# NicolaDM/MAPLE

Measured on AMD Instinct MI355X. Metric: candidate SPR placements/sec, higher is better.
Workload: dtype f64

## Files before the change

### include/maple_hip.h

```cpp
#ifndef MAPLE_HIP_H
#define MAPLE_HIP_H
#include <stdint.h>

#ifdef __cplusplus
extern "C" {
#endif

#define MAPLE_ABI_VERSION 4

enum {
    MAPLE_OK = 0,
    MAPLE_ERR_ARG = -1,
    MAPLE_ERR_HIP = -2,
    MAPLE_ERR_NOMEM = -3,
    MAPLE_ERR_STATE = -4,
    MAPLE_ERR_FATAL = -5
};

#define MAPLE_META_TYPE(m)   ((m) & 7u)
#define MAPLE_META_REF(m)    (((m) >> 3) & 3u)
#define MAPLE_META_HASD0     (1u << 5)
#define MAPLE_META_HASD1     (1u << 6)
#define MAPLE_META_FLAG      (1u << 7)
#define MAPLE_META_AUXOFF(m) ((m) >> 8)
// ... 4 lines not shown
    double thresholdProb;
    double minBLenSensitivity;
    double thresholdDiffForUpdate;
    double thresholdFoldChangeUpdate;
    double defaultBLen;
} maple_params;

int maple_abi_version(void);
int maple_create(maple_ctx **out, int device, int32_t lRef, const uint8_t *refIdx,
                 const double *rootFreqs4, const maple_params *params, uint64_t arena_bytes);
int maple_destroy(maple_ctx *ctx);
typedef struct {
    uint32_t structSize;
    int32_t wavePerItemMax;
    int32_t placementChunkMax;
    int32_t noCladeScan;
    int32_t verbose;
    int32_t wideOutsideFrontier;
    int32_t denseWideScoring;
    int32_t waveAllBelow;
    int32_t noOverHint;
    int32_t noAheadExpansion;
    int32_t noAheadSpeculation;
} maple_tuning;
int maple_set_tuning(maple_ctx *ctx, const maple_tuning *t);
const char *maple_last_error(maple_ctx *ctx);

int maple_set_model(maple_ctx *ctx, const double *Q16, const double *siteRates, int usingErrorRate,
                    double errorRateGlobal, const double *errorRates);
int maple_get_model(maple_ctx *ctx, double *cumulativeRate , double *cumulativeErrorRate ,
                    double *totError);

int maple_lists_update(maple_ctx *ctx, int32_t n, const int32_t *ids, const int64_t *ent_off, const int32_t *pos,
                       const uint32_t *meta, const int64_t *aux_off, const double *aux);
int maple_lists_upload(maple_ctx *ctx, int32_t n_lists, const int64_t *ent_off, const int32_t *pos,
                       const uint32_t *meta, const int64_t *aux_off, const double *aux, int32_t *first_id);
int maple_lists_sizes(maple_ctx *ctx, int32_t n, const int32_t *ids, int32_t *n_ent, int32_t *n_aux);
int maple_lists_download(maple_ctx *ctx, int32_t n, const int32_t *ids, const int64_t *ent_off, int32_t *pos,
                         uint32_t *meta, const int64_t *aux_off, double *aux);
int maple_arena_mark(maple_ctx *ctx, int64_t *mark);
int maple_arena_release(maple_ctx *ctx, int64_t mark);
int maple_arena_stats(maple_ctx *ctx, int64_t *n_lists, int64_t *n_entries, int64_t *n_aux, int64_t *cap_entries);
int maple_arena_compact(maple_ctx *ctx, int64_t nLive, const int32_t *live, int32_t *newIds);

int maple_mutations_upload(maple_ctx *ctx, int32_t n_lists, const int64_t *off, const int32_t *mut3,
                           int32_t *first_id);
// ... 110 lines not shown
```

### include/maple_hip_debug.h

```cpp
#ifndef MAPLE_HIP_DEBUG_H
#define MAPLE_HIP_DEBUG_H
#include "maple_hip.h"

#ifdef __cplusplus
extern "C" {
#endif

int maple_debug_frontier_levels(maple_ctx *ctx, int32_t cap, int64_t *itemsUpdating, int64_t *itemsCached, float *msUpdating,
                                float *msCached, int32_t *n, int64_t *waveItemsSmall , int64_t *waveItemsBig );

int maple_debug_wave_append_batch(maple_ctx *ctx, int32_t n, const int32_t *parentList, const int32_t *childList,
                                  const uint8_t *isTipC, const double *bLen, double *outLK, float *ms);
int maple_debug_trace_query(maple_ctx *ctx, int32_t query);
int maple_debug_calib_walk(maple_ctx *ctx, uint64_t bytes, int32_t repeats, float *ms);
int maple_debug_calib_write(maple_ctx *ctx, uint64_t bytes, int32_t mode, int32_t repeats, float *ms);
int maple_debug_trace_read(maple_ctx *ctx, int32_t *n, int32_t *items4 , double *vals2 );
int maple_debug_gpv_batch(maple_ctx *ctx, int32_t n, const int32_t *i12, const double *totLen, const double *M16,
                          const double *errorRate, const double *vect4, const uint8_t *upNode, const uint8_t *flag,
                          double *out4);
int maple_debug_simplify_batch(maple_ctx *ctx, int32_t n, const double *vec4, const int32_t *refA, int32_t *out);
int maple_debug_frontier_pass_batch(maple_ctx *ctx, int32_t n, const int32_t *list, const int32_t *mutList, const uint8_t *dirIsUp,
                                    int32_t waveForm, int32_t *outList, uint8_t *grade, uint8_t *sameHandle);

#ifdef __cplusplus
}
#endif
#endif
```

### maple_amd/csrc/debug_abi.hip

```cpp
#include "../../include/maple_hip_debug.h"
#include "genome_dev.h"
#include "ctx_host.h"
#include "batch_host.h"
#include "frontier.h"
#include "frontier_dev.h"

#include <algorithm>

using namespace frt;

__global__ __launch_bounds__(MAPLE_BLOCK) void k_calib_walk(const unsigned long long *buf, long long nLists, unsigned long long *sink)
{
    unsigned long long acc = 0;
    for (long long l = (long long)blockIdx.x * blockDim.x + threadIdx.x; l < nLists; l += (long long)gridDim.x * blockDim.x) {
        const unsigned long long *p = buf + l * 64;
        unsigned idx = 0;
        for (int k = 0; k < 64; k++) {
            unsigned long long w = p[idx];
            acc += w;
            idx = (idx + 1 + (unsigned)(w & 0)) & 63;
        }
    }
    if (acc == 0x123456789abcdefull) *sink = acc;
}
// ... 146 lines not shown

extern "C" int maple_debug_trace_query(maple_ctx *c, int32_t query)
{
    if (!c) return MAPLE_ERR_ARG;
    c->trace_query = query;
    if (query >= 0) {
        HIPCK(c, c->s_trace_i.reserve(4 * 4096 + 4));
        HIPCK(c, c->s_trace_d.reserve(2 * 4096));
        HIPCK(c, hipMemset(c->s_trace_i.p, 0, (4 * 4096 + 4) * sizeof(int32_t)));
    }
    return MAPLE_OK;
}

extern "C" int maple_debug_trace_read(maple_ctx *c, int32_t *n, int32_t *items4, double *vals2)
{
    if (!c || !n || !items4 || !vals2 || !c->s_trace_i.p) return MAPLE_ERR_ARG;
    HIPCK(c, hipMemcpy(n, c->s_trace_i.p + 4 * 4096, sizeof(int32_t), hipMemcpyDeviceToHost));
    HIPCK(c, hipMemcpy(items4, c->s_trace_i.p, 4 * 4096 * sizeof(int32_t), hipMemcpyDeviceToHost));
    HIPCK(c, hipMemcpy(vals2, c->s_trace_d.p, 2 * 4096 * sizeof(double), hipMemcpyDeviceToHost));
    return MAPLE_OK;
}

extern "C" int maple_debug_frontier_levels(maple_ctx *c, int32_t cap, int64_t *itemsUpdating, int64_t *itemsCached, float *msUpdating,
                                           float *msCached, int32_t *n, int64_t *waveItemsSmall, int64_t *waveItemsBig)
{
    if (!c || cap < 0 || !itemsUpdating || !itemsCached || !msUpdating || !msCached || !n) return MAPLE_ERR_ARG;
    HIPCK(c, hipSetDevice(c->device));
    int nn = 0;
    const int rc = frontier_level_profile(c, cap, (long long *)itemsUpdating, (long long *)itemsCached, msUpdating, msCached, &nn,
                                          (long long *)waveItemsSmall, (long long *)waveItemsBig);
    *n = nn;
    return rc;
}

template <bool RV, bool U, bool SS>
__global__ __launch_bounds__(FR_BLOCK) void k_debug_fpass_lane(const DevModel *__restrict__ mp, ArenaViewS av, FPools fp, int n, const int32_t *l,
                                                               const int32_t *ml, const uint8_t *up, int32_t *handle)
{
    __shared__ Lds lds;
    const DevModel &m = *mp;
    stage_model(m, lds);
    Ctx<RV, U, SS> c(m, lds);
    const long long laneId = (long long)blockIdx.x * blockDim.x + threadIdx.x;
    for (long long i = laneId; i < n; i += (long long)gridDim.x * blockDim.x)
        handle[i] = fpass_removed(c, fp, av, laneId, ftree(l[i]), ml[i], up[i] != 0);
}

template <bool RV, bool U, bool SS>
__global__ __launch_bounds__(FR_BLOCK) void k_debug_fpass_wave(const DevModel *__restrict__ mp, ArenaViewS av, FPools fp, int n, const int32_t *l,
                                                               const int32_t *ml, const uint8_t *up, int32_t *handle)
{
    __shared__ Lds lds;
    const DevModel &m = *mp;
// ... 95 lines not shown
```

### maple_amd/csrc/frontier.h

```cpp
#pragma once
#include "ctx_host.h"

#define FR_STATUS_FALLBACK (-8)

struct FrontierStats {
    int levels = 0, overflow = 0;
    long long itemsUpdating = 0, itemsCached = 0, tempLists = 0, tempWords = 0, tempAux = 0, records = 0;
};

struct FrontierWide {
    const int32_t *rowOf;
    const double *cacheS;
    FiniteRows fin;
    hipEvent_t rowsReady;
    int forceWide;
    const int32_t *frameParent = nullptr, *frameNode = nullptr;
    int nFrames = 0;
};

__attribute__((visibility("hidden")))
int frontier_search(maple_ctx *c, const SearchParams &P, int m, const int32_t *nodes, int budget, int zeroBudget, SearchOut *hostOut,
                    uint2 *poolW, double *poolA, unsigned long long *poolUsed, long long poolCapW, long long poolCapA,
                    FrontierStats *stats, long long itemsHint, const FrontierWide *wide = nullptr,
                    const uint8_t *overHint = nullptr);
__attribute__((visibility("hidden"))) void frontier_scratch_free(maple_ctx *c);
__attribute__((visibility("hidden"))) int frontier_export(maple_ctx *c, long long cap, int32_t *q, int32_t *node, long long *n);
__attribute__((visibility("hidden")))
int frontier_level_profile(maple_ctx *c, int cap, long long *itemsU, long long *itemsC, float *msU, float *msC, int *n,
                           long long *waveSmall = nullptr, long long *waveBig = nullptr);
```

### maple_amd/csrc/frontier.hip

```cpp
#include "ctx_host.h"
#include "frontier_dev.h"

#include <chrono>

using namespace frt;

namespace {

__global__ __launch_bounds__(FR_BLOCK) void k_fr_arena_recs(ArenaViewS av, int n, LRec *out)
{
    for (int i = blockIdx.x * blockDim.x + threadIdx.x; i < n; i += gridDim.x * blockDim.x)
        out[i] = lrec_make(av.ent_off[i], av.n_ent[i], av.aux_off[i], av.n_aux[i]);
}

template <bool RV, bool U, bool SS>
__global__ __launch_bounds__(FR_BLOCK) void k_fr_begin(const DevModel *__restrict__ mp, ArenaViewS av, DevTree T, SearchParams P, int n,
                                                       const int32_t *nodes, FPools fp, SearchOut *out, int budget, int zeroBudget,
                                                       const int32_t *rowOf, int forceWide, const uint8_t *overHint)
{
    __shared__ Lds lds;
    const DevModel &m = *mp;
    stage_model(m, lds);
    Ctx<RV, U, SS> c(m, lds);
    for (int q = blockIdx.x * blockDim.x + threadIdx.x; q < n; q += gridDim.x * blockDim.x) {
// ... 63 lines not shown
        const int pp = rp.up;
        const NodeRec rpp = T.nd[pp];
        const bool first = rpp.c0 == parent;
        const double d = rs.dist + rp.dist;
        int pv1 = ftree(rs.lower), rprUp = rpr, vUpUp = ftree(first ? rpp.upRight : rpp.upLeft), rprDown = rpr;
        if (fp.mat) {
            pv1 = fpass_store(fp, av, c.m.lRef, laneId, pv1, rs.mutId, true);
            if (rp.mutId >= 0) {
                pv1 = fvalid(pv1) ? fpass_store(fp, av, c.m.lRef, laneId, pv1, rp.mutId, true) : pv1;
                rprUp = fpass_removed(c, fp, av, laneId, rpr, rp.mutId, true);
            }
            vUpUp = fpass_store(fp, av, c.m.lRef, laneId, vUpUp, rp.mutId, false);
            if (rs.mutId >= 0) {
                vUpUp = fvalid(vUpUp) ? fpass_store(fp, av, c.m.lRef, laneId, vUpUp, rs.mutId, false) : vUpUp;
                rprDown = hBest;
            }
            if (pv1 == -2 || vUpUp == -2 || !fvalid(rprUp) || !fvalid(rprDown)) { S.state = FS_FALLBACK; continue; }
        }
        S.seed0 = fpush(fp, budget, q, true, pp, first ? 1 : 2, pv1, d, curLK, 0, rprUp, curLK);
        S.seed1 = fpush(fp, budget, q, true, S.sibling, 0, vUpUp, d, curLK, 0, rprDown, curLK);
    }
}

#define FR_LVL 8
__global__ void k_fr_snap_u(FCtr *ctr, long long capU, long long capR, long long capPassR, unsigned long long *lvl, int maxLevels)
{
    if (threadIdx.x == 0 && blockIdx.x == 0) {
        ctr->loU = ctr->hiU; ctr->hiU = min(ctr->usedU, (unsigned long long)capU);
        atomicExch(&ctr->safePassR, min(ctr->nPassR, (unsigned long long)capPassR));
        __threadfence();
        atomicExch(&ctr->safeR, min(ctr->usedR, (unsigned long long)capR));
        ctr->bigUsed = 0;
        const unsigned long long heavySmall = ctr->permHeavy, heavyBig = ctr->permHeavy2;
        ctr->permDown = ctr->permUp = ctr->permDownB = ctr->permUpB = ctr->permHeavy = ctr->permHeavy2 = 0;
        if (lvl) {
            const int l = ctr->nLevels++;
            if (l < maxLevels) { lvl[FR_LVL * l] = ctr->loU; lvl[FR_LVL * l + 1] = ctr->hiU; lvl[FR_LVL * l + 6] = lvl[FR_LVL * l + 7] = 0; }
            if (l > 0 && l - 1 < maxLevels) { lvl[FR_LVL * (l - 1) + 6] = heavySmall; lvl[FR_LVL * (l - 1) + 7] = heavyBig; }
        }
    }
}
__global__ void k_fr_snap_c(FCtr *ctr, long long capCC, long long capPass, long long capDeferred, unsigned long long *lvl, int maxLevels)
{
    if (threadIdx.x == 0 && blockIdx.x == 0) {
        ctr->loC = ctr->hiC; ctr->hiC = min(ctr->usedC, (unsigned long long)capCC);
        ctr->loR = ctr->hiR; ctr->hiR = atomicAdd(&ctr->safeR, 0ull);
// ... 248 lines not shown
                atomicAdd(&fp.ctr->dbgC[2], (unsigned long long)(tp2 - tp1)); atomicAdd(&fp.ctr->dbgC[3], (unsigned long long)(tp3 - tp2));
                atomicAdd(&fp.ctr->dbgC[4], (unsigned long long)len); atomicAdd(&fp.ctr->dbgC[5], (unsigned long long)nS);
                atomicAdd(&fp.ctr->dbgC[6], (unsigned long long)tot);
            }
        }
#endif
    }
    for (int off = 32; off > 0; off >>= 1) {
        nSc += ((unsigned long long)(uint32_t)__shfl_down((int)(nSc >> 32), off, 64) << 32) | (uint32_t)__shfl_down((int)nSc, off, 64);
        bSc += ((unsigned long long)(uint32_t)__shfl_down((int)(bSc >> 32), off, 64) << 32) | (uint32_t)__shfl_down((int)bSc, off, 64);
    }
    if ((threadIdx.x & 63) == 0 && nSc) { atomicAdd(&fp.ctr->scoredC, nSc); atomicAdd(&fp.ctr->bytesC, bSc); }
}

__device__ __forceinline__ long long fidx(const FPools &fp, int ref) { return ref >= 0 ? fp.capU + ref : -(long long)(ref + 2); }
__device__ __forceinline__ int fsize(const FPools &fp, int ref) { return ref == FR_NONE ? 0 : fp.lsize[fidx(fp, ref)]; }

__device__ __forceinline__ void fr_layer(const FPools &fp, int level, int which, long long &lo1, long long &n1, long long &lo2, long long &n2)
{
    const unsigned long long *L = fp.lvl + (size_t)FR_LVL * level;
    if (which == 0) { lo1 = (long long)L[0]; n1 = (long long)L[1] - lo1; lo2 = 0; n2 = 0; }
    else { lo1 = (long long)L[2]; n1 = (long long)L[3] - lo1; lo2 = (long long)L[4]; n2 = (long long)L[5] - lo2; }
}
__global__ __launch_bounds__(FR_BLOCK) void k_fr_layout_sizes(FPools fp, int level, int which)
{
    long long lo1, n1, lo2, n2;
    fr_layer(fp, level, which, lo1, n1, lo2, n2);
    const long long n = n1 + n2;
    const bool isU = which == 0;
    for (long long i = (long long)blockIdx.x * blockDim.x + threadIdx.x; i < n; i += (long long)gridDim.x * blockDim.x) {
        const long long at = i < n1 ? lo1 + i : lo2 + (i - n1);
        const FItem &it = isU ? fp.U[at] : fp.C[at];
        fp.lsize[isU ? at : fp.capU + at] = 1 + fsize(fp, it.child0) + fsize(fp, it.child1);
    }
}
__global__ __launch_bounds__(FR_BLOCK) void k_fr_layout_totals(int n, FPools fp)
{
    for (int q = blockIdx.x * blockDim.x + threadIdx.x; q < n; q += gridDim.x * blockDim.x) {
        const FSearch &S = fp.S[q];
        fp.tot[q] = S.state == FS_ACTIVE ? fsize(fp, S.seed0) + fsize(fp, S.seed1) : 0;
    }
}
__global__ __launch_bounds__(1024) void k_fr_layout_scan(int n, const int32_t *in, long long *out)
{
    __shared__ long long part[1024];
    const int t = threadIdx.x, per = (n + 1023) / 1024;
    const int lo = min(n, t * per), hi = min(n, lo + per);
    long long s = 0;
    for (int i = lo; i < hi; i++) s += in[i];
    part[t] = s;
    __syncthreads();
    if (t == 0) {
        long long run = 0;
        for (int i = 0; i < 1024; i++) { const long long v = part[i]; part[i] = run; run += v; }
        out[n] = run;
    }
    __syncthreads();
    long long run = part[t];
    for (int i = lo; i < hi; i++) { out[i] = run; run += in[i]; }
}
__global__ __launch_bounds__(FR_BLOCK) void k_fr_layout_seeds(int n, FPools fp)
{
    for (int q = blockIdx.x * blockDim.x + threadIdx.x; q < n; q += gridDim.x * blockDim.x) {
        const FSearch &S = fp.S[q];
        if (S.state != FS_ACTIVE || fp.vbase[q + 1] > fp.capVisit) continue;
        long long p = fp.vbase[q];
        if (S.seed1 != FR_NONE) { const long long x = fidx(fp, S.seed1); fp.lpos[x] = (int32_t)p; fp.lpar[x] = -1; p += fp.lsize[x]; }
        if (S.seed0 != FR_NONE) { const long long x = fidx(fp, S.seed0); fp.lpos[x] = (int32_t)p; fp.lpar[x] = -1; }
    }
}
__global__ __launch_bounds__(FR_BLOCK) void k_fr_layout_place(FPools fp, int level, int which)
{
    long long lo1, n1, lo2, n2;
    fr_layer(fp, level, which, lo1, n1, lo2, n2);
    const long long n = n1 + n2;
    const bool isU = which == 0;
    for (long long i = (long long)blockIdx.x * blockDim.x + threadIdx.x; i < n; i += (long long)gridDim.x * blockDim.x) {
        const long long at = i < n1 ? lo1 + i : lo2 + (i - n1);
        const long long own = isU ? at : fp.capU + at;
        const int p = fp.lpos[own];
        if (p < 0) continue;
        const FItem &it = isU ? fp.U[at] : fp.C[at];
        FVisit v;
        v.midProb = it.midProb; v.lastLK = it.lastLK; v.ref = isU ? -((int)at + 2) : (int)at; v.size = fp.lsize[own];
        v.parent = fp.lpar[own]; v.flags = it.flags; v.dir = it.dir; v.failsOut = 0;
        fp.visit[p] = v;
        int q = p + 1;
        if (it.child1 != FR_NONE) { const long long x = fidx(fp, it.child1); fp.lpos[x] = q; fp.lpar[x] = p; q += fp.lsize[x]; }
        if (it.child0 != FR_NONE) { const long long x = fidx(fp, it.child0); fp.lpos[x] = q; fp.lpar[x] = p; }
    }
}

__device__ inline void fr_replay_done(const SearchParams &P, const FPools &fp, SearchOut *out, int q, FSearch &S, int slHead, int nApp, bool handBack,
                                      const int *hShort = nullptr, int nShort = 0, int reason = 0)
{
    for (int k = 0; k < nShort; k++) if (hShort[k] == S.hRpr0 && !handBack) { handBack = true; reason = 4; }
    if (handBack) { S.state = FS_FALLBACK; out[q].status = FR_STATUS_FALLBACK; atomicAdd(&fp.ctr->fbReason[reason & 7], 1); return; }
    S.slHead = slHead; S.nApp = nApp;
    int cnt = 0;
    for (int r = slHead; r != FR_NONE; r = item_of(fp, r).next)
        if (item_of(fp, r).midProb >= S.curLK - P.thrOptTopo) cnt++;
    const unsigned long long base = atomicAdd(&fp.ctr->nRecs, (unsigned long long)cnt);
    if ((long long)(base + cnt) > fp.capRecs) {
        S.state = FS_FALLBACK; out[q].status = FR_STATUS_FALLBACK; fp.ctr->overflow = 1;
        for (long long k2 = (long long)base; k2 < fp.capRecs; k2++) { fp.recs[k2].q = q; fp.recs[k2].ref = FR_NONE; }
        return;
    }
    S.recBase = (int32_t)base; S.recCount = cnt;
    int k = 0;
    for (int r = slHead; r != FR_NONE; r = item_of(fp, r).next)
        if (item_of(fp, r).midProb >= S.curLK - P.thrOptTopo) {
            FRec &x = fp.recs[base + k++];
// ... 449 lines not shown
__global__ __launch_bounds__(FR_BLOCK) void k_fr_export(FPools fp, long long nU, long long nC, long long nR, int32_t *outQ, int32_t *outNode)
{
    const long long n = nU + nC + nR;
    for (long long i = (long long)blockIdx.x * blockDim.x + threadIdx.x; i < n; i += (long long)gridDim.x * blockDim.x) {
        const FItem &it = i < nU ? fp.U[i] : (i < nU + nC ? fp.C[i - nU] : fp.C[fp.capCC + (i - nU - nC)]);
        outQ[i] = it.q; outNode[i] = it.t1;
    }
}

struct FrontierScratch {
    DevBuf<uint8_t> itemsU, itemsC, srch, recs, ctr;
    DevBuf<uint2> tw, sw, bw;
    DevBuf<double> ta, sa, sais, ba;
    DevBuf<LRec> trec, arec;
    DevBuf<int32_t> nodes, expQ, expNode;
    DevBuf<uint8_t> out, wideBr, tflag, overHint;
    DevBuf<int32_t> wideRow, wideQ, wideCtr, perm, perm2, perm3, perm4, tot, lsize, lpos, lpar, passList, passListR, deferred;
    DevBuf<uint2> bw2; DevBuf<double> ba2;
    DevBuf<uint8_t> visit;
    DevBuf<unsigned long long> lvl;
    DevBuf<long long> vbase;
    std::vector<unsigned long long> lastLvl;
    std::vector<size_t> lastSlotsU, lastSlotsC;
    long long lastU = -1, lastC = -1, lastR = 0;
    long long needR = 0;
    long long needU = 0, needC = 0, needL = 0, needW = 0, needA = 0, needM = 0;
    bool lastOverflow = false;
    FPools lastPools{};
    int capE = 0;
    hipStream_t side = nullptr, side2 = nullptr;
    hipEvent_t evFork = nullptr, evJoin = nullptr, evFork2 = nullptr, evJoin2 = nullptr;
};

}

void frontier_scratch_free(maple_ctx *c)
{
    FrontierScratch *F = (FrontierScratch *)c->frontier;
    if (!F) return;
    F->itemsU.release(); F->itemsC.release(); F->srch.release(); F->recs.release(); F->ctr.release();
    F->tw.release(); F->sw.release(); F->ta.release(); F->sa.release(); F->sais.release(); F->bw.release(); F->ba.release();
    F->trec.release(); F->arec.release(); F->nodes.release(); F->out.release();
    F->expQ.release(); F->expNode.release();
    F->perm.release(); F->perm2.release(); F->perm3.release(); F->perm4.release(); F->tot.release(); F->lsize.release(); F->lpos.release(); F->lpar.release(); F->visit.release(); F->lvl.release(); F->vbase.release(); F->wideBr.release(); F->wideRow.release(); F->wideQ.release(); F->wideCtr.release(); F->passList.release(); F->passListR.release(); F->deferred.release(); F->overHint.release(); F->bw2.release(); F->ba2.release(); F->tflag.release();
    if (F->evFork) (void)hipEventDestroy(F->evFork);
    if (F->evJoin) (void)hipEventDestroy(F->evJoin);
// ... 261 lines not shown
        launchesC++;
        return MAPLE_OK;
    };
    auto bail = [&](int rc) { (void)hipStreamSynchronize(s); (void)hipStreamSynchronize(s2); (void)hipStreamSynchronize(s3); return rc; };
    k_fr_snap_u<<<1, 64, 0, s>>>(fp.ctr, fp.capU, fp.capC - fp.capCC, fp.capPassR, fp.lvl, fp.maxLevels);
    if (hipGetLastError() != hipSuccess || hipEventRecord(F.evFork, s) != hipSuccess || hipStreamWaitEvent(s2, F.evFork, 0) != hipSuccess
        || (anyWide && wide->rowsReady && hipStreamWaitEvent(s2, wide->rowsReady, 0) != hipSuccess))
        return bail(fail(c, MAPLE_ERR_HIP, "frontier level loop: HIP error"));
    const int groupLevels = m <= 64 ? 2 : 8;
    for (;;) {
        for (int g = 0; g < groupLevels; g++) {
            { const int rc_ = u_level(); if (rc_) return bail(rc_); }
            for (int k2 = 0; k2 < 2; k2++) { const int rc_ = c_launch(); if (rc_) return bail(rc_); }
        }
        if (hipGetLastError() != hipSuccess || hipMemcpyAsync(&hc, fp.ctr, sizeof(FCtr), hipMemcpyDeviceToHost, s) != hipSuccess
            || hipStreamSynchronize(s) != hipSuccess)
            return bail(fail(c, MAPLE_ERR_HIP, "frontier level loop: HIP error"));
        if (hc.hiU == hc.loU) break;
        if (levels > 100000) return bail(fail(c, MAPLE_ERR_FATAL, "frontier search did not terminate"));
    }
    for (;;) {
        for (int g = 0; g < groupLevels; g++) { const int rc_ = c_launch(); if (rc_) return bail(rc_); }
        if (passQueued && hipStreamWaitEvent(s2, F.evJoin2, 0) != hipSuccess) return bail(fail(c, MAPLE_ERR_HIP, "frontier level loop: HIP error"));
        if (hipGetLastError() != hipSuccess || hipMemcpyAsync(&hc, fp.ctr, sizeof(FCtr), hipMemcpyDeviceToHost, s2) != hipSuccess
            || hipStreamSynchronize(s2) != hipSuccess)
            return bail(fail(c, MAPLE_ERR_HIP, "frontier level loop: HIP error"));
        const unsigned long long haveC = std::min<unsigned long long>(hc.usedC, (unsigned long long)fp.capCC),
                                 haveR = std::min<unsigned long long>(hc.usedR, (unsigned long long)(fp.capC - fp.capCC));
        if (hc.hiC == haveC && hc.hiR == haveR && hc.hiD == std::min<unsigned long long>(hc.nDeferred, (unsigned long long)fp.capDeferred)) break;
        if (launchesC > 200000) return bail(fail(c, MAPLE_ERR_FATAL, "frontier search did not terminate"));
    }
    if (hipEventRecord(F.evJoin, s2) != hipSuccess || hipStreamWaitEvent(s, F.evJoin, 0) != hipSuccess)
        return bail(fail(c, MAPLE_ERR_HIP, "frontier level loop: HIP error"));
    if (dbgTime) fprintf(stderr, "[maple]   frontier +%.1f ms: expansion done (%d updating levels, %d cached launches)\n", sinceEnter(), levels, launchesC);
    size_t slotWide = (size_t)-1;
    auto finishStage = [&]() -> int {
    if (anyWide) {
        hipEvent_t w0, w1;
        TRY(maple_internal_ev_pair(c, &w0, &w1, MAPLE_K_FR_WIDE, 0.0, 0.0));
        slotWide = c->ev_used / 2 - 1;
        const int capB = 512, gridW = (int)std::min<size_t>(8192, wideIdx.size());
        HIPCK(c, F.wideBr.reserve_exact(std::max(F.wideBr.cap, (size_t)gridW * capB * sizeof(BestRec))));
        HIPCK(c, hipEventRecord(F.evFork, s));
        HIPCK(c, hipStreamWaitEvent(s2, F.evFork, 0));
        HIPCK(c, hipEventRecord(w0, s2));
        const size_t dyn = (size_t)Tw.scanDepthCap * (sizeof(double) + sizeof(int) + sizeof(unsigned));
        k_fr_replay_wide<<<gridW, 64, dyn, s2>>>(Tw, P, (int)wideIdx.size(), F.wideQ.p, F.wideRow.p, wide->cacheS, wide->fin, fp, dout,
                                                  (BestRec *)F.wideBr.p, capB, F.wideCtr.p);
        HIPCK(c, hipGetLastError());
        HIPCK(c, hipEventRecord(w1, s2));
        HIPCK(c, hipEventRecord(F.evJoin, s2));
    }
    TRY(maple_internal_ev_pair(c, &er0, &er1, MAPLE_K_FR_REPLAY, (double)m, 0.0));
    HIPCK(c, hipEventRecord(er0, s));
    const int gridLayout = (int)std::min<long long>(1024, std::max<long long>(64, (long long)m / 64));
    if (levels <= fp.maxLevels && launchesC <= fp.maxLevels && fp.visit) {
        HIPCK(c, hipMemsetAsync(fp.lpos, 0xFF, (size_t)fp.capVisit * sizeof(int32_t), s));
        for (int l = launchesC - 1; l >= 0; l--) k_fr_layout_sizes<<<gridLayout, FR_BLOCK, 0, s>>>(fp, l, 1);
        for (int l = levels - 1; l >= 0; l--) k_fr_layout_sizes<<<gridLayout, FR_BLOCK, 0, s>>>(fp, l, 0);
        k_fr_layout_totals<<<gridN, FR_BLOCK, 0, s>>>(m, fp);
        k_fr_layout_scan<<<1, 1024, 0, s>>>(m, fp.tot, fp.vbase);
        k_fr_layout_seeds<<<gridN, FR_BLOCK, 0, s>>>(m, fp);
        for (int l = 0; l < levels; l++) k_fr_layout_place<<<gridLayout, FR_BLOCK, 0, s>>>(fp, l, 0);
        for (int l = 0; l < launchesC; l++) k_fr_layout_place<<<gridLayout, FR_BLOCK, 0, s>>>(fp, l, 1);
        HIPCK(c, hipGetLastError());
        TRY(stage("k_fr_layout"));
    } else fp.visit = nullptr;
    k_fr_replay<<<gridN, FR_BLOCK, 0, s>>>(P, m, fp, dout);
    TRY(stage("k_fr_replay"));
    if (anyWide) HIPCK(c, hipStreamWaitEvent(s, F.evJoin, 0));
    if (anyWide && fp.mat && wide->nFrames > 0) {
        DISPATCH3(c, k_fr_wide_frames, <<<std::min(gridUpd, 512), FR_BLOCK, 0, s>>>(c->d_model, av, T, fp, wide->frameParent, wide->frameNode));
        TRY(stage("k_fr_wide_frames"));
    }
    DISPATCH3(c, k_fr_refine, <<<gridUpd, FR_BLOCK, 0, s>>>(c->d_model, av, T, fp));
    TRY(stage("k_fr_refine"));
    k_fr_finish<<<gridN, FR_BLOCK, 0, s>>>(av, T, P, m, fp, dout, poolW, poolA, poolUsed, poolCapW, poolCapA);
    HIPCK(c, hipGetLastError());
    HIPCK(c, hipEventRecord(er1, s));
    HIPCK(c, hipEventRecord(e1, s));
    HIPCK(c, hipMemcpyAsync(hostOut, dout, (size_t)m * sizeof(SearchOut), hipMemcpyDeviceToHost, s));
    HIPCK(c, hipMemcpyAsync(&hc, fp.ctr, sizeof(FCtr), hipMemcpyDeviceToHost, s));
    HIPCK(c, hipStreamSynchronize(s));
    return MAPLE_OK;
    };
    { const int rc_ = finishStage(); if (rc_) return bail(rc_); }
    if (dbgTime) fprintf(stderr, "[maple]   frontier +%.1f ms: replay, refinement, final selection done; results on the host\n", sinceEnter());
    if (dbgTime && (hc.fbReason[0] | hc.fbReason[1] | hc.fbReason[2] | hc.fbReason[3] | hc.fbReason[4] | hc.fbReason[5] | hc.fbReason[6] | hc.fbReason[7]))
        fprintf(stderr, "[maple]   exact walk handed searches to the one-lane kernel: %d a merge within tolerance, %d a list re-expressed from a shortened one, "
                        "%d a fifth shortened list, %d the search's own first list shortened, %d marked list without a layout, %d other; whole-tree searches: "
                        "%d short list / scan slots / marked item list, %d a scanned branch whose list shorten() would change\n",
                hc.fbReason[1], hc.fbReason[2], hc.fbReason[3], hc.fbReason[4], hc.fbReason[5], hc.fbReason[0], hc.fbReason[6], hc.fbReason[7]);
    if (dbgTime && hc.overflow)
        fprintf(stderr, "[maple]   frontier pools, asked / capacity: updating items %llu / %lld, cached items %llu / %lld, roots %llu / %lld, temporary lists %llu / %lld "
                        "(words %llu / %lld, aux %llu / %lld), pass entries %llu / %lld, of roots %llu / %lld, records %llu / %lld\n",
                hc.usedU, fp.capU, hc.usedC, fp.capCC, hc.usedR, fp.capC - fp.capCC, hc.nLists, fp.capL, hc.usedW, fp.capW, hc.usedA, fp.capA,
                hc.nPass, fp.capPass, hc.nPassR, fp.capPassR, hc.nRecs, fp.capRecs);
    {
        const double meanCand = c->n_scored ? c->scored_bytes_total / c->n_scored : 0.0;
        double units = 0.0, bytes = 0.0;
        double unitsW = 0.0, bytesW = 0.0;
        for (int k = 0; k < m; k++) {
            if (hostOut[k].status != 0 && hostOut[k].status != -1) continue;
            if (anyWide && wide->rowOf[k] >= 0) {
                const int32_t l = c->h_tree_lower[nodes[k]];
                unitsW += hostOut[k].nAppend;
                bytesW += 8.0 * hostOut[k].nAppend + (l >= 0 ? 8.0 * c->h_n_ent[l] + 8.0 * c->h_n_aux[l] : 0.0);
                continue;
            }
            units += hostOut[k].nAppend;
// ... 21 lines not shown
    {
        const char *nm[4] = {"small class", "512 class", "small class, one lane (a list does not fit)", "512 class, one lane (a list does not fit)"};
        for (int b = 0; b < 4; b++)
            if (hc.dbgWCnt[b]) fprintf(stderr, "[maple] wavefront-wide updating items, %s: %llu items, mean %.3f ms, slowest %.3f ms\n", nm[b],
                                       hc.dbgWCnt[b], hc.dbgWT[b] * 1e-5 / hc.dbgWCnt[b], hc.dbgWMax[b] * 1e-5);
    }
    if (anyWide) {
        double tw = 0, ts = 0, mw = 0, ms = 0; long long ns = 0, mxn = 0;
        for (int k : wideIdx) {
            tw += hostOut[k].tStep * 1e-5; ts += hostOut[k].tReplay * 1e-5; ns += hostOut[k].nSteps;
            mw = std::max(mw, hostOut[k].tStep * 1e-5); ms = std::max(ms, hostOut[k].tReplay * 1e-5); mxn = std::max<long long>(mxn, hostOut[k].nSteps);
        }
        fprintf(stderr, "[maple] wide replay profile over %zu searches: item walk %.1f ms total (max %.2f), scans %.1f ms total (max %.2f), %lld scans (max %lld)\n",
                wideIdx.size(), tw, mw, ts, ms, ns, mxn);
    }
#endif
    if (!(anyWide && wide->forceWide) && (m >= 1024 || m >= F.needM)) {
        F.needU = (long long)hc.usedU; F.needC = (long long)hc.usedC; F.needR = (long long)hc.usedR; F.needL = (long long)hc.nLists; F.needW = (long long)hc.usedW;
        F.needA = (long long)hc.usedA; F.needM = m; F.lastOverflow = hc.overflow != 0;
    }
    F.lastU = std::min((long long)hc.usedU, fp.capU); F.lastC = std::min((long long)hc.usedC, fp.capCC);
    F.lastR = std::min((long long)hc.usedR, fp.capC - fp.capCC); F.lastPools = fp;
    {
        const int nl = std::min(std::max(levels, launchesC), fp.maxLevels);
        F.lastLvl.assign((size_t)nl * FR_LVL, 0ull);
        if (nl) HIPCK(c, hipMemcpy(F.lastLvl.data(), fp.lvl, (size_t)nl * FR_LVL * sizeof(unsigned long long), hipMemcpyDeviceToHost));
        for (int l = 0; l < nl; l++) {
            unsigned long long *L = F.lastLvl.data() + (size_t)FR_LVL * l;
            if (l >= levels) L[0] = L[1] = L[6] = L[7] = 0;
            if (l >= launchesC) L[2] = L[3] = L[4] = L[5] = 0;
        }
        F.lastSlotsU = slotsU; F.lastSlotsC = slotsC;
    }
    if (hc.overflow) F.lastU = F.lastC = -1;
    if (stats) {
        stats->levels = levels; stats->itemsUpdating = (long long)hc.usedU; stats->itemsCached = (long long)(hc.usedC + hc.usedR);
        stats->tempLists = (long long)hc.nLists; stats->tempWords = (long long)hc.usedW; stats->tempAux = (long long)hc.usedA;
        stats->records = (long long)hc.nRecs; stats->overflow = hc.overflow;
    }
    return MAPLE_OK;
}

int frontier_export(maple_ctx *c, long long cap, int32_t *q, int32_t *node, long long *n)
{
    FrontierScratch *F = (FrontierScratch *)c->frontier;
    if (!F || F->lastU < 0) return fail(c, MAPLE_ERR_STATE, "no complete frontier search to export");
    const long long tot = F->lastU + F->lastC + F->lastR;
    *n = tot;
    if (tot > cap) return fail(c, MAPLE_ERR_ARG, "%lld expanded items do not fit in %lld", tot, cap);
    if (tot == 0) return MAPLE_OK;
    HIPCK(c, F->expQ.reserve((size_t)tot));
    HIPCK(c, F->expNode.reserve((size_t)tot));
    k_fr_export<<<(int)std::min<long long>(1024, (tot + FR_BLOCK - 1) / FR_BLOCK), FR_BLOCK, 0, c->stream>>>(F->lastPools, F->lastU, F->lastC, F->lastR,
                                                                                                          F->expQ.p, F->expNode.p);
    HIPCK(c, hipGetLastError());
    HIPCK(c, hipMemcpyAsync(q, F->expQ.p, (size_t)tot * sizeof(int32_t), hipMemcpyDeviceToHost, c->stream));
    HIPCK(c, hipMemcpyAsync(node, F->expNode.p, (size_t)tot * sizeof(int32_t), hipMemcpyDeviceToHost, c->stream));
    HIPCK(c, hipStreamSynchronize(c->stream));
    return MAPLE_OK;
}

int frontier_level_profile(maple_ctx *c, int cap, long long *itemsU, long long *itemsC, float *msU, float *msC, int *n, long long *waveSmall,
                           long long *waveBig)
{
    FrontierScratch *F = (FrontierScratch *)c->frontier;
    if (!F) return fail(c, MAPLE_ERR_STATE, "no frontier search to report on");
    const int nl = (int)(F->lastLvl.size() / FR_LVL);
    *n = nl;
    for (int l = 0; l < nl && l < cap; l++) {
        const unsigned long long *L = F->lastLvl.data() + (size_t)FR_LVL * l;
        itemsU[l] = (long long)(L[1] - L[0]);
        itemsC[l] = (long long)(L[3] - L[2]) + (long long)(L[5] - L[4]);
        if (waveSmall) waveSmall[l] = (long long)L[6];
        if (waveBig) waveBig[l] = (long long)L[7];
        msU[l] = msC[l] = 0.f;
        const size_t su = l < (int)F->lastSlotsU.size() ? F->lastSlotsU[l] : (size_t)-1 / 4, sc = l < (int)F->lastSlotsC.size() ? F->lastSlotsC[l] : (size_t)-1 / 4;
        if (2 * su + 1 < c->ev_used) { HIPCK(c, hipEventSynchronize(c->evs[2 * su + 1])); HIPCK(c, hipEventElapsedTime(&msU[l], c->evs[2 * su], c->evs[2 * su + 1])); }
        if (2 * sc + 1 < c->ev_used) { HIPCK(c, hipEventSynchronize(c->evs[2 * sc + 1])); HIPCK(c, hipEventElapsedTime(&msC[l], c->evs[2 * sc], c->evs[2 * sc + 1])); }
    }
    return MAPLE_OK;
}
```

### maple_amd/runtime.py

```python
from __future__ import annotations

import ctypes as C
import os

import numpy as np

from .genome_list import PackedLists, pack_lists, pack_mutations, unpack_list

HERE = os.path.dirname(os.path.abspath(__file__))
LIB_PATH = os.path.join(HERE, "libmaple_hip.so")

EXPORTS = [
    "maple_abi_version", "maple_create", "maple_destroy", "maple_set_tuning", "maple_last_error", "maple_set_model", "maple_get_model",
    "maple_lists_upload", "maple_lists_update", "maple_lists_sizes", "maple_lists_download", "maple_arena_mark", "maple_arena_release",
    "maple_arena_stats", "maple_mutations_upload", "maple_append_batch", "maple_merge_batch", "maple_blen_batch",
    "maple_differ_batch", "maple_pass_branch_batch", "maple_shorten_batch", "maple_root_vector_batch",
    "maple_evaluate_placement_batch", "maple_update_partials", "maple_update_partials_touched", "maple_tree_patch", "maple_append_batch_dev", "maple_append_queries_dev", "maple_timing_reset", "maple_timing_read", "maple_timing_read_each",
    "maple_append_algorithmic_bytes", "maple_tree_upload", "maple_spr_search_batch", "maple_minor_batch", "maple_root_prob_batch", "maple_candset_create", "maple_append_candset",
    "maple_minor_candset", "maple_placement_search_batch", "maple_placement_prepare", "maple_placement_ahead", "maple_placement_ahead_stats", "maple_set_fatal_policy",
    "maple_timing_read_kind", "maple_placement_supports_batch",
    "maple_candset_destroy", "maple_spr_search_visited", "maple_arena_compact", "maple_append_queries_argmax_dev", "maple_comm_unique_id", "maple_comm_init", "maple_argmax_allreduce_dev", "maple_tree_rebuild_lists",
]


DEBUG_EXPORTS = ["maple_debug_wave_append_batch", "maple_debug_trace_query", "maple_debug_trace_read", "maple_debug_calib_walk",
                 "maple_debug_calib_write", "maple_debug_gpv_batch", "maple_debug_simplify_batch", "maple_debug_frontier_levels",
                 "maple_debug_frontier_pass_batch"]
LIB_PATH_DEBUG = os.path.join(HERE, "libmaple_hip_debug.so")


class MapleParams(C.Structure):
    _fields_ = [("thresholdProb", C.c_double), ("minBLenSensitivity", C.c_double),
                ("thresholdDiffForUpdate", C.c_double), ("thresholdFoldChangeUpdate", C.c_double),
                ("defaultBLen", C.c_double)]


class MapleSearchParams(C.Structure):
    _fields_ = [("strictTopologyStopRules", C.c_int32), ("allowedFailsTopology", C.c_int32),
                ("thresholdLogLKtopology", C.c_double), ("thresholdTopologyPlacement", C.c_double),
                ("thresholdLogLKoptimizationTopology", C.c_double), ("thresholdLogLKconsecutivePlacement", C.c_double),
                ("effectivelyNon0BLen", C.c_double), ("wideSearchBudget", C.c_int32), ("searchTier", C.c_int32)]


class MapleTuning(C.Structure):
    _fields_ = [("structSize", C.c_uint32), ("wavePerItemMax", C.c_int32), ("placementChunkMax", C.c_int32), ("noCladeScan", C.c_int32), ("verbose", C.c_int32),
                ("wideOutsideFrontier", C.c_int32), ("denseWideScoring", C.c_int32), ("waveAllBelow", C.c_int32), ("noOverHint", C.c_int32), ("noAheadExpansion", C.c_int32), ("noAheadSpeculation", C.c_int32)]


class MaplePlacementParams(C.Structure):
    _fields_ = [("oneMutBLen", C.c_double), ("effectivelyNon0BLen", C.c_double), ("thresholdLogLK", C.c_double),
                ("thresholdLogLKoptimization", C.c_double), ("thresholdLogLKconsecutivePlacement", C.c_double),
                ("allowedFails", C.c_int32), ("strictStopRules", C.c_int32), ("onlyFindIdentical", C.c_int32)]


class MapleError(RuntimeError):
    ERR_ARG, ERR_HIP, ERR_NOMEM, ERR_STATE, ERR_FATAL = -1, -2, -3, -4, -5

    def __init__(self, msg, code=None):
        super().__init__(msg)
        self.code = code


_lib = None
_lib_debug = None


def load_library(debug=False):
    global _lib, _lib_debug
    if (_lib_debug if debug else _lib) is None:
# ... 54 lines not shown
            raise MapleError(f"maple_create failed ({rc}): no usable MI355X / HIP runtime; the placement path has no "
                             "CPU fallback")
        self.h = h
        self.device = int(device)
        self.u = False

    def _ck(self, rc):
        if rc != 0:
            msg = self.lib.maple_last_error(self.h)
            raise MapleError(f"libmaple_hip error {rc}: {msg.decode() if msg else ''}", rc)

    def close(self):
        if getattr(self, "h", None):
            self.lib.maple_destroy(self.h)
            self.h = None

    def __del__(self):
        try:
            self.close()
        except Exception:
            pass

    def set_tuning(self, *, wave_per_item_max=0, placement_chunk_max=0, no_clade_scan=False, verbose=0, wide_outside_frontier=False,
                   dense_wide_scoring=False, wave_all_below=0, no_over_hint=False, no_ahead_expansion=False, no_ahead_speculation=False):
        t = MapleTuning(C.sizeof(MapleTuning), int(wave_per_item_max), int(placement_chunk_max), int(bool(no_clade_scan)), int(verbose),
                        int(bool(wide_outside_frontier)), int(bool(dense_wide_scoring)), int(wave_all_below), int(bool(no_over_hint)),
                        int(no_ahead_expansion), int(bool(no_ahead_speculation)))
        self._ck(self.lib.maple_set_tuning(self.h, C.byref(t)))

    def set_model(self, Q, siteRates=None, usingErrorRate=False, errorRateGlobal=0.0, errorRates=None):
        Qf = _f64(np.asarray(Q, dtype=np.float64).reshape(16))
        sr = None if siteRates is None else _f64(siteRates)
        er = None if (errorRates is None or not usingErrorRate) else _f64(errorRates)
        self._ck(self.lib.maple_set_model(self.h, _ptr(Qf), _ptr(sr), int(bool(usingErrorRate)),
                                          C.c_double(errorRateGlobal or 0.0), _ptr(er)))
        self.u = bool(usingErrorRate)

    def get_model(self):
        cr = np.zeros(self.lRef + 1)
        ce = np.zeros(self.lRef + 1)
        te = C.c_double()
        self._ck(self.lib.maple_get_model(self.h, _ptr(cr), _ptr(ce), C.byref(te)))
        return cr, ce, te.value

    def upload_packed(self, pl: PackedLists):
        first = C.c_int32()
        self._ck(self.lib.maple_lists_upload(self.h, len(pl), _ptr(pl.ent_off), _ptr(pl.pos), _ptr(pl.meta),
                                             _ptr(pl.aux_off), _ptr(pl.aux), C.byref(first)))
        return np.arange(first.value, first.value + len(pl), dtype=np.int32)

# ... 388 lines not shown
        self._ck(self.lib.maple_comm_unique_id(self.h, _ptr(buf)))
        return buf

    def comm_init(self, world, rank, unique_id):
        self._ck(self.lib.maple_comm_init(self.h, int(world), int(rank), _ptr(_u8(unique_id))))

    def argmax_allreduce_dev(self, n, score_ptr, idx_ptr, stream=0):
        self._ck(self.lib.maple_argmax_allreduce_dev(self.h, int(n), C.c_void_p(score_ptr), C.c_void_p(idx_ptr), C.c_void_p(stream)))

    def timing_reset(self):
        self._ck(self.lib.maple_timing_reset(self.h))

    def timing_read_each(self, cap=256):
        ms = np.zeros(cap, dtype=np.float32)
        n = C.c_int32()
        self._ck(self.lib.maple_timing_read_each(self.h, int(cap), _ptr(ms), C.byref(n)))
        return ms[: n.value].tolist()

    def frontier_levels(self, cap=4096):
        iu, ic = np.zeros(cap, np.int64), np.zeros(cap, np.int64)
        ws, wb = np.zeros(cap, np.int64), np.zeros(cap, np.int64)
        mu, mc = np.zeros(cap, np.float32), np.zeros(cap, np.float32)
        n = C.c_int32()
        self._ck(self.lib.maple_debug_frontier_levels(self.h, int(cap), _ptr(iu), _ptr(ic), _ptr(mu), _ptr(mc), C.byref(n), _ptr(ws), _ptr(wb)))
        k = min(cap, n.value)
        self.last_wave_items = (ws[:k], wb[:k])
        return iu[:k], ic[:k], mu[:k], mc[:k]

    def tree_rebuild_lists(self, root, up, c0, c1, tip, mut, dist, lower, bump_len=0.0):
        n = len(up)
        up, c0, c1 = _i32(up), _i32(c0), _i32(c1)
        tip = np.ascontiguousarray(np.asarray(tip, np.uint8))
        mutp = None if mut is None else _i32(mut)
        assert dist.dtype == np.float64 and dist.flags.c_contiguous
        lower = _i32(lower).copy()
        ur, ul, tu = (np.full(n, -1, np.int32) for _ in range(3))
        bad = np.zeros(max(64, n), np.int32)
        nbad = C.c_int32()
        self._ck(self.lib.maple_tree_rebuild_lists(self.h, n, int(root), _ptr(up), _ptr(c0), _ptr(c1), _ptr(tip), _ptr(mutp), _ptr(dist),
                                                   _ptr(lower), _ptr(ur), _ptr(ul), _ptr(tu), C.c_double(bump_len), len(bad), _ptr(bad),
                                                   C.byref(nbad)))
        return lower, ur, ul, tu, np.unique(bad[: min(nbad.value, len(bad))])

    def timing_read(self):
        n, ms = C.c_int32(), C.c_double()
        self._ck(self.lib.maple_timing_read(self.h, C.byref(n), C.byref(ms)))
        return n.value, ms.value

# ... 16 lines not shown
```

Baseline: 42.37 billion.

## Fuse small frontier layout layers into single-block kernels to cut launch count

Reads per-level item counts back to the host alongside the existing counter copy, then groups consecutive small layout layers (below a tunable threshold) into one single-block kernel that walks them in order with __syncthreads between layers. Large layers keep their per-layer grid launches. The lpos memset is replaced by resetting lpos inside the size pass. The aim is to remove the many tiny kernel launches in deep trees, at the cost of serialising small layers onto one block and an extra async copy before the sync.

```diff
diff --git a/include/maple_hip.h b/include/maple_hip.h
--- a/include/maple_hip.h
+++ b/include/maple_hip.h
@@ -50,6 +50,7 @@
     int32_t noOverHint;
     int32_t noAheadExpansion;
     int32_t noAheadSpeculation;
+    int32_t layoutFuseBelow;
 } maple_tuning;
 int maple_set_tuning(maple_ctx *ctx, const maple_tuning *t);
 const char *maple_last_error(maple_ctx *ctx);
diff --git a/include/maple_hip_debug.h b/include/maple_hip_debug.h
--- a/include/maple_hip_debug.h
+++ b/include/maple_hip_debug.h
@@ -7,7 +7,8 @@
 #endif
 
 int maple_debug_frontier_levels(maple_ctx *ctx, int32_t cap, int64_t *itemsUpdating, int64_t *itemsCached, float *msUpdating,
-                                float *msCached, int32_t *n, int64_t *waveItemsSmall , int64_t *waveItemsBig );
+                                float *msCached, int32_t *n, int64_t *waveItemsSmall , int64_t *waveItemsBig ,
+                                int32_t *layout3 );
 
 int maple_debug_wave_append_batch(maple_ctx *ctx, int32_t n, const int32_t *parentList, const int32_t *childList,
                                   const uint8_t *isTipC, const double *bLen, double *outLK, float *ms);
diff --git a/maple_amd/csrc/debug_abi.hip b/maple_amd/csrc/debug_abi.hip
--- a/maple_amd/csrc/debug_abi.hip
+++ b/maple_amd/csrc/debug_abi.hip
@@ -192,13 +192,13 @@
 }
 
 extern "C" int maple_debug_frontier_levels(maple_ctx *c, int32_t cap, int64_t *itemsUpdating, int64_t *itemsCached, float *msUpdating,
-                                           float *msCached, int32_t *n, int64_t *waveItemsSmall, int64_t *waveItemsBig)
+                                           float *msCached, int32_t *n, int64_t *waveItemsSmall, int64_t *waveItemsBig, int32_t *layout3)
 {
     if (!c || cap < 0 || !itemsUpdating || !itemsCached || !msUpdating || !msCached || !n) return MAPLE_ERR_ARG;
     HIPCK(c, hipSetDevice(c->device));
     int nn = 0;
     const int rc = frontier_level_profile(c, cap, (long long *)itemsUpdating, (long long *)itemsCached, msUpdating, msCached, &nn,
-                                          (long long *)waveItemsSmall, (long long *)waveItemsBig);
+                                          (long long *)waveItemsSmall, (long long *)waveItemsBig, layout3);
     *n = nn;
     return rc;
 }
diff --git a/maple_amd/csrc/frontier.h b/maple_amd/csrc/frontier.h
--- a/maple_amd/csrc/frontier.h
+++ b/maple_amd/csrc/frontier.h
@@ -27,4 +27,4 @@
 __attribute__((visibility("hidden"))) int frontier_export(maple_ctx *c, long long cap, int32_t *q, int32_t *node, long long *n);
 __attribute__((visibility("hidden")))
 int frontier_level_profile(maple_ctx *c, int cap, long long *itemsU, long long *itemsC, float *msU, float *msC, int *n,
-                           long long *waveSmall = nullptr, long long *waveBig = nullptr);
+                           long long *waveSmall = nullptr, long long *waveBig = nullptr, int *layout = nullptr);
diff --git a/maple_amd/csrc/frontier.hip b/maple_amd/csrc/frontier.hip
--- a/maple_amd/csrc/frontier.hip
+++ b/maple_amd/csrc/frontier.hip
@@ -109,6 +109,9 @@
     }
 }
 
+#ifndef FR_LAYOUT_FUSE_BELOW
+#define FR_LAYOUT_FUSE_BELOW 8192
+#endif
 #define FR_LVL 8
 __global__ void k_fr_snap_u(FCtr *ctr, long long capU, long long capR, long long capPassR, unsigned long long *lvl, int maxLevels)
 {
@@ -403,17 +406,20 @@
     if (which == 0) { lo1 = (long long)L[0]; n1 = (long long)L[1] - lo1; lo2 = 0; n2 = 0; }
     else { lo1 = (long long)L[2]; n1 = (long long)L[3] - lo1; lo2 = (long long)L[4]; n2 = (long long)L[5] - lo2; }
 }
+__device__ __forceinline__ void fr_layout_size_item(const FPools &fp, bool isU, long long at)
+{
+    const FItem &it = isU ? fp.U[at] : fp.C[at];
+    const long long own = isU ? at : fp.capU + at;
+    fp.lsize[own] = 1 + fsize(fp, it.child0) + fsize(fp, it.child1);
+    fp.lpos[own] = -1;
+}
 __global__ __launch_bounds__(FR_BLOCK) void k_fr_layout_sizes(FPools fp, int level, int which)
 {
     long long lo1, n1, lo2, n2;
     fr_layer(fp, level, which, lo1, n1, lo2, n2);
     const long long n = n1 + n2;
-    const bool isU = which == 0;
-    for (long long i = (long long)blockIdx.x * blockDim.x + threadIdx.x; i < n; i += (long long)gridDim.x * blockDim.x) {
-        const long long at = i < n1 ? lo1 + i : lo2 + (i - n1);
-        const FItem &it = isU ? fp.U[at] : fp.C[at];
-        fp.lsize[isU ? at : fp.capU + at] = 1 + fsize(fp, it.child0) + fsize(fp, it.child1);
-    }
+    for (long long i = (long long)blockIdx.x * blockDim.x + threadIdx.x; i < n; i += (long long)gridDim.x * blockDim.x)
+        fr_layout_size_item(fp, which == 0, i < n1 ? lo1 + i : lo2 + (i - n1));
 }
 __global__ __launch_bounds__(FR_BLOCK) void k_fr_layout_totals(int n, FPools fp)
 {
@@ -450,25 +456,42 @@
         if (S.seed0 != FR_NONE) { const long long x = fidx(fp, S.seed0); fp.lpos[x] = (int32_t)p; fp.lpar[x] = -1; }
     }
 }
+__device__ __forceinline__ void fr_layout_place_item(const FPools &fp, bool isU, long long at)
+{
+    const long long own = isU ? at : fp.capU + at;
+    const int p = fp.lpos[own];
+    if (p < 0) return;
+    const FItem &it = isU ? fp.U[at] : fp.C[at];
+    FVisit v;
+    v.midProb = it.midProb; v.lastLK = it.lastLK; v.ref = isU ? -((int)at + 2) : (int)at; v.size = fp.lsize[own];
+    v.parent = fp.lpar[own]; v.flags = it.flags; v.dir = it.dir; v.failsOut = 0;
+    fp.visit[p] = v;
+    int q = p + 1;
+    if (it.child1 != FR_NONE) { const long long x = fidx(fp, it.child1); fp.lpos[x] = q; fp.lpar[x] = p; q += fp.lsize[x]; }
+    if (it.child0 != FR_NONE) { const long long x = fidx(fp, it.child0); fp.lpos[x] = q; fp.lpar[x] = p; }
+}
 __global__ __launch_bounds__(FR_BLOCK) void k_fr_layout_place(FPools fp, int level, int which)
 {
     long long lo1, n1, lo2, n2;
     fr_layer(fp, level, which, lo1, n1, lo2, n2);
     const long long n = n1 + n2;
-    const bool isU = which == 0;
-    for (long long i = (long long)blockIdx.x * blockDim.x + threadIdx.x; i < n; i += (long long)gridDim.x * blockDim.x) {
-        const long long at = i < n1 ? lo1 + i : lo2 + (i - n1);
-        const long long own = isU ? at : fp.capU + at;
-        const int p = fp.lpos[own];
-        if (p < 0) continue;
-        const FItem &it = isU ? fp.U[at] : fp.C[at];
-        FVisit v;
-        v.midProb = it.midProb; v.lastLK = it.lastLK; v.ref = isU ? -((int)at + 2) : (int)at; v.size = fp.lsize[own];
-        v.parent = fp.lpar[own]; v.flags = it.flags; v.dir = it.dir; v.failsOut = 0;
-        fp.visit[p] = v;
-        int q = p + 1;
-        if (it.child1 != FR_NONE) { const long long x = fidx(fp, it.child1); fp.lpos[x] = q; fp.lpar[x] = p; q += fp.lsize[x]; }
-        if (it.child0 != FR_NONE) { const long long x = fidx(fp, it.child0); fp.lpos[x] = q; fp.lpar[x] = p; }
+    for (long long i = (long long)blockIdx.x * blockDim.x + threadIdx.x; i < n; i += (long long)gridDim.x * blockDim.x)
+        fr_layout_place_item(fp, which == 0, i < n1 ? lo1 + i : lo2 + (i - n1));
+}
+__global__ __launch_bounds__(1024) void k_fr_layout_fused(FPools fp, int pass, int first, int count, int levels, int launchesC)
+{
+    for (int sq = first; sq < first + count; sq++) {
+        int which, level;
+        if (pass == 0) { which = sq < launchesC ? 1 : 0; level = which ? launchesC - 1 - sq : levels - 1 - (sq - launchesC); }
+        else { which = sq < levels ? 0 : 1; level = which ? sq - levels : sq; }
+        long long lo1, n1, lo2, n2;
+        fr_layer(fp, level, which, lo1, n1, lo2, n2);
+        const long long n = n1 + n2;
+        for (long long i = threadIdx.x; i < n; i += blockDim.x) {
+            const long long at = i < n1 ? lo1 + i : lo2 + (i - n1);
+            if (pass == 0) fr_layout_size_item(fp, which == 0, at); else fr_layout_place_item(fp, which == 0, at);
+        }
+        __syncthreads();
     }
 }
 
@@ -964,6 +987,7 @@
     DevBuf<long long> vbase;
     std::vector<unsigned long long> lastLvl;
     std::vector<size_t> lastSlotsU, lastSlotsC;
+    int lastLayout[3] = {0, 0, 0};
     long long lastU = -1, lastC = -1, lastR = 0;
     long long needR = 0;
     long long needU = 0, needC = 0, needL = 0, needW = 0, needA = 0, needM = 0;
@@ -1271,6 +1295,10 @@
     for (;;) {
         for (int g = 0; g < groupLevels; g++) { const int rc_ = c_launch(); if (rc_) return bail(rc_); }
         if (passQueued && hipStreamWaitEvent(s2, F.evJoin2, 0) != hipSuccess) return bail(fail(c, MAPLE_ERR_HIP, "frontier level loop: HIP error"));
+        const int nl = std::min(std::max(levels, launchesC), fp.maxLevels);
+        F.lastLvl.resize((size_t)nl * FR_LVL);
+        if (hipMemcpyAsync(F.lastLvl.data(), fp.lvl, (size_t)nl * FR_LVL * sizeof(unsigned long long), hipMemcpyDeviceToHost, s2) != hipSuccess)
+            return bail(fail(c, MAPLE_ERR_HIP, "frontier level loop: HIP error"));
         if (hipGetLastError() != hipSuccess || hipMemcpyAsync(&hc, fp.ctr, sizeof(FCtr), hipMemcpyDeviceToHost, s2) != hipSuccess
             || hipStreamSynchronize(s2) != hipSuccess)
             return bail(fail(c, MAPLE_ERR_HIP, "frontier level loop: HIP error"));
@@ -1283,6 +1311,7 @@
         return bail(fail(c, MAPLE_ERR_HIP, "frontier level loop: HIP error"));
     if (dbgTime) fprintf(stderr, "[maple]   frontier +%.1f ms: expansion done (%d updating levels, %d cached launches)\n", sinceEnter(), levels, launchesC);
     size_t slotWide = (size_t)-1;
+    int layoutLaunches = 0;
     auto finishStage = [&]() -> int {
     if (anyWide) {
         hipEvent_t w0, w1;
@@ -1303,15 +1332,40 @@
     TRY(maple_internal_ev_pair(c, &er0, &er1, MAPLE_K_FR_REPLAY, (double)m, 0.0));
     HIPCK(c, hipEventRecord(er0, s));
     const int gridLayout = (int)std::min<long long>(1024, std::max<long long>(64, (long long)m / 64));
+    layoutLaunches = 0;
     if (levels <= fp.maxLevels && launchesC <= fp.maxLevels && fp.visit) {
-        HIPCK(c, hipMemsetAsync(fp.lpos, 0xFF, (size_t)fp.capVisit * sizeof(int32_t), s));
-        for (int l = launchesC - 1; l >= 0; l--) k_fr_layout_sizes<<<gridLayout, FR_BLOCK, 0, s>>>(fp, l, 1);
-        for (int l = levels - 1; l >= 0; l--) k_fr_layout_sizes<<<gridLayout, FR_BLOCK, 0, s>>>(fp, l, 0);
+        const long long fuseBelow = c->tuning.layoutFuseBelow > 0 ? c->tuning.layoutFuseBelow : (c->tuning.layoutFuseBelow < 0 ? -1 : FR_LAYOUT_FUSE_BELOW);
+        const int nSeq = levels + launchesC;
+        auto layerOf = [&](int pass, int sq, int &which, int &level) {
+            if (pass == 0) { which = sq < launchesC ? 1 : 0; level = which ? launchesC - 1 - sq : levels - 1 - (sq - launchesC); }
+            else { which = sq < levels ? 0 : 1; level = which ? sq - levels : sq; }
+        };
+        auto itemsOf = [&](int which, int level) -> long long {
+            const unsigned long long *L = F.lastLvl.data() + (size_t)FR_LVL * level;
+            return which == 0 ? (long long)(L[1] - L[0]) : (long long)(L[3] - L[2]) + (long long)(L[5] - L[4]);
+        };
+        auto runPass = [&](int pass) {
+            for (int sq = 0; sq < nSeq;) {
+                int which, level;
+                layerOf(pass, sq, which, level);
+                if (itemsOf(which, level) > fuseBelow) {
+                    if (pass == 0) k_fr_layout_sizes<<<gridLayout, FR_BLOCK, 0, s>>>(fp, level, which);
+                    else k_fr_layout_place<<<gridLayout, FR_BLOCK, 0, s>>>(fp, level, which);
+                    sq++;
+                } else {
+                    int e = sq + 1;
+                    for (; e < nSeq; e++) { layerOf(pass, e, which, level); if (itemsOf(which, level) > fuseBelow) break; }
+                    k_fr_layout_fused<<<1, 1024, 0, s>>>(fp, pass, sq, e - sq, levels, launchesC);
+                    sq = e;
+                }
+                layoutLaunches++;
+            }
+        };
+        runPass(0);
         k_fr_layout_totals<<<gridN, FR_BLOCK, 0, s>>>(m, fp);
         k_fr_layout_scan<<<1, 1024, 0, s>>>(m, fp.tot, fp.vbase);
         k_fr_layout_seeds<<<gridN, FR_BLOCK, 0, s>>>(m, fp);
-        for (int l = 0; l < levels; l++) k_fr_layout_place<<<gridLayout, FR_BLOCK, 0, s>>>(fp, l, 0);
-        for (int l = 0; l < launchesC; l++) k_fr_layout_place<<<gridLayout, FR_BLOCK, 0, s>>>(fp, l, 1);
+        runPass(1);
         HIPCK(c, hipGetLastError());
         TRY(stage("k_fr_layout"));
     } else fp.visit = nullptr;
@@ -1334,7 +1388,8 @@
     return MAPLE_OK;
     };
     { const int rc_ = finishStage(); if (rc_) return bail(rc_); }
-    if (dbgTime) fprintf(stderr, "[maple]   frontier +%.1f ms: replay, refinement, final selection done; results on the host\n", sinceEnter());
+    if (dbgTime) fprintf(stderr, "[maple]   frontier +%.1f ms: replay, refinement, final selection done; results on the host (layout: %d launches over 2 x %d layers; %llu records refined)\n",
+                         sinceEnter(), layoutLaunches, levels + launchesC, hc.nRecs);
     if (dbgTime && (hc.fbReason[0] | hc.fbReason[1] | hc.fbReason[2] | hc.fbReason[3] | hc.fbReason[4] | hc.fbReason[5] | hc.fbReason[6] | hc.fbReason[7]))
         fprintf(stderr, "[maple]   exact walk handed searches to the one-lane kernel: %d a merge within tolerance, %d a list re-expressed from a shortened one, "
                         "%d a fifth shortened list, %d the search's own first list shortened, %d marked list without a layout, %d other; whole-tree searches: "
@@ -1402,15 +1457,14 @@
     F.lastU = std::min((long long)hc.usedU, fp.capU); F.lastC = std::min((long long)hc.usedC, fp.capCC);
     F.lastR = std::min((long long)hc.usedR, fp.capC - fp.capCC); F.lastPools = fp;
     {
-        const int nl = std::min(std::max(levels, launchesC), fp.maxLevels);
-        F.lastLvl.assign((size_t)nl * FR_LVL, 0ull);
-        if (nl) HIPCK(c, hipMemcpy(F.lastLvl.data(), fp.lvl, (size_t)nl * FR_LVL * sizeof(unsigned long long), hipMemcpyDeviceToHost));
+        const int nl = (int)(F.lastLvl.size() / FR_LVL);
         for (int l = 0; l < nl; l++) {
             unsigned long long *L = F.lastLvl.data() + (size_t)FR_LVL * l;
             if (l >= levels) L[0] = L[1] = L[6] = L[7] = 0;
             if (l >= launchesC) L[2] = L[3] = L[4] = L[5] = 0;
         }
         F.lastSlotsU = slotsU; F.lastSlotsC = slotsC;
+        F.lastLayout[0] = layoutLaunches; F.lastLayout[1] = levels; F.lastLayout[2] = launchesC;
     }
     if (hc.overflow) F.lastU = F.lastC = -1;
     if (stats) {
@@ -1441,10 +1495,11 @@
 }
 
 int frontier_level_profile(maple_ctx *c, int cap, long long *itemsU, long long *itemsC, float *msU, float *msC, int *n, long long *waveSmall,
-                           long long *waveBig)
+                           long long *waveBig, int *layout)
 {
     FrontierScratch *F = (FrontierScratch *)c->frontier;
     if (!F) return fail(c, MAPLE_ERR_STATE, "no frontier search to report on");
+    if (layout) for (int k = 0; k < 3; k++) layout[k] = F->lastLayout[k];
     const int nl = (int)(F->lastLvl.size() / FR_LVL);
     *n = nl;
     for (int l = 0; l < nl && l < cap; l++) {
diff --git a/maple_amd/runtime.py b/maple_amd/runtime.py
--- a/maple_amd/runtime.py
+++ b/maple_amd/runtime.py
@@ -44,7 +44,8 @@
 
 class MapleTuning(C.Structure):
     _fields_ = [("structSize", C.c_uint32), ("wavePerItemMax", C.c_int32), ("placementChunkMax", C.c_int32), ("noCladeScan", C.c_int32), ("verbose", C.c_int32),
-                ("wideOutsideFrontier", C.c_int32), ("denseWideScoring", C.c_int32), ("waveAllBelow", C.c_int32), ("noOverHint", C.c_int32), ("noAheadExpansion", C.c_int32), ("noAheadSpeculation", C.c_int32)]
+                ("wideOutsideFrontier", C.c_int32), ("denseWideScoring", C.c_int32), ("waveAllBelow", C.c_int32), ("noOverHint", C.c_int32), ("noAheadExpansion", C.c_int32), ("noAheadSpeculation", C.c_int32),
+                ("layoutFuseBelow", C.c_int32)]
 
 
 class MaplePlacementParams(C.Structure):
@@ -145,10 +146,11 @@
             pass
 
     def set_tuning(self, *, wave_per_item_max=0, placement_chunk_max=0, no_clade_scan=False, verbose=0, wide_outside_frontier=False,
-                   dense_wide_scoring=False, wave_all_below=0, no_over_hint=False, no_ahead_expansion=False, no_ahead_speculation=False):
+                   dense_wide_scoring=False, wave_all_below=0, no_over_hint=False, no_ahead_expansion=False, no_ahead_speculation=False,
+                   layout_fuse_below=0):
         t = MapleTuning(C.sizeof(MapleTuning), int(wave_per_item_max), int(placement_chunk_max), int(bool(no_clade_scan)), int(verbose),
                         int(bool(wide_outside_frontier)), int(bool(dense_wide_scoring)), int(wave_all_below), int(bool(no_over_hint)),
-                        int(no_ahead_expansion), int(bool(no_ahead_speculation)))
+                        int(no_ahead_expansion), int(bool(no_ahead_speculation)), int(layout_fuse_below))
         self._ck(self.lib.maple_set_tuning(self.h, C.byref(t)))
 
     def set_model(self, Q, siteRates=None, usingErrorRate=False, errorRateGlobal=0.0, errorRates=None):
@@ -583,8 +585,11 @@
         ws, wb = np.zeros(cap, np.int64), np.zeros(cap, np.int64)
         mu, mc = np.zeros(cap, np.float32), np.zeros(cap, np.float32)
         n = C.c_int32()
-        self._ck(self.lib.maple_debug_frontier_levels(self.h, int(cap), _ptr(iu), _ptr(ic), _ptr(mu), _ptr(mc), C.byref(n), _ptr(ws), _ptr(wb)))
+        lay = np.zeros(3, np.int32)
+        self._ck(self.lib.maple_debug_frontier_levels(self.h, int(cap), _ptr(iu), _ptr(ic), _ptr(mu), _ptr(mc), C.byref(n), _ptr(ws), _ptr(wb),
+                                                      _ptr(lay)))
         k = min(cap, n.value)
+        self.last_layout = tuple(int(x) for x in lay)
         self.last_wave_items = (ws[:k], wb[:k])
         return iu[:k], ic[:k], mu[:k], mc[:k]
 
```

Result: faster. 42.92 billion (median of 6 runs) (+1.3%).
